# QEDProtocol/plonky2.5

Hardware: NVIDIA B200
Metric: commit Melem/s (2^20x135 LDE+Poseidon Merkle) (higher is better)
Workload: dtype u64 (Goldilocks field, integer + exact fp64 limb arithmetic)

## Files before the change

### plonky2.5_b200/csrc/merkle.cuh

```cuda
#pragma once
#include "poseidon.cuh"

namespace merkle {

__host__ __device__ __forceinline__ uint64_t digest_index(uint32_t layer, uint64_t j) {
    return 2 * (((j >> 1) << (layer + 1)) + (1ULL << layer) - 1) + (j & 1);
}

__device__ __forceinline__ void store_digest(uint64_t* dst, const uint64_t (&s)[poseidon::WIDTH]) {
    ulonglong2* d = reinterpret_cast<ulonglong2*>(dst);
    d[0] = make_ulonglong2(gl::canon(s[0]), gl::canon(s[1]));
    d[1] = make_ulonglong2(gl::canon(s[2]), gl::canon(s[3]));
}

#ifndef LEAF_MIN_BLOCKS
#define LEAF_MIN_BLOCKS 6
#endif
template <int BLOCK>
__global__ void __launch_bounds__(BLOCK, LEAF_MIN_BLOCKS)
leaf_hash_kernel(const uint64_t* __restrict__ leaves, uint32_t pitch, uint32_t leaf_len, uint64_t n_leaves,
                 uint32_t log_sub, uint64_t* __restrict__ digests, uint64_t* __restrict__ cap) {
    uint64_t leaf = (uint64_t)blockIdx.x * BLOCK + threadIdx.x;
    if (leaf >= n_leaves) return;
    const uint64_t* row = leaves + leaf * pitch;
    uint64_t s[poseidon::WIDTH];
#pragma unroll
    for (int i = 0; i < poseidon::WIDTH; i++) s[i] = 0;
    if (leaf_len <= 4) {
#pragma unroll
        for (int i = 0; i < 4; i++)
            if ((uint32_t)i < leaf_len) s[i] = row[i];
    } else {
        const uint32_t n_chunks = (leaf_len + 7) >> 3;
#pragma unroll 1
        for (uint32_t k = 0; k < n_chunks; k++) {
            const ulonglong2* src = reinterpret_cast<const ulonglong2*>(row + 8 * k);
            ulonglong2 v0 = __ldg(src), v1 = __ldg(src + 1), v2 = __ldg(src + 2), v3 = __ldg(src + 3);
            uint64_t in[8] = {v0.x, v0.y, v1.x, v1.y, v2.x, v2.y, v3.x, v3.y};
            const uint32_t rem = leaf_len - 8 * k;
#pragma unroll
            for (int i = 0; i < 8; i++)
                if ((uint32_t)i < rem) s[i] = in[i];
            poseidon::permute(s);
        }
    }
    uint64_t* dst;
    if (log_sub == 0) dst = cap + 4 * leaf;
    else {
        uint64_t L = 1ULL << log_sub, t = leaf >> log_sub, j = leaf & (L - 1);
        dst = digests + 4 * (t * 2 * (L - 1) + digest_index(0, j));
    }
    store_digest(dst, s);
}

template <int BLOCK>
__global__ void __launch_bounds__(BLOCK, LEAF_MIN_BLOCKS)
leaf_absorb_kernel(const uint64_t* __restrict__ leaves, uint32_t pitch, uint32_t leaf_len, uint32_t col0, uint32_t col1, uint64_t n_leaves,
                   uint32_t log_sub, uint64_t* __restrict__ state, uint64_t* __restrict__ digests, uint64_t* __restrict__ cap, int first, int last) {
    const uint64_t leaf = (uint64_t)blockIdx.x * BLOCK + threadIdx.x;
    if (leaf >= n_leaves) return;
    const uint64_t* row = leaves + leaf * pitch;
    uint64_t s[poseidon::WIDTH];
    const bool in_full = leaf_len - col0 >= 8;
#pragma unroll
    for (int i = 0; i < poseidon::WIDTH; i++) s[i] = (first || (i < 8 && in_full)) ? 0 : state[(uint64_t)i * n_leaves + leaf];
#pragma unroll 1
    for (uint32_t k = col0; k < col1; k += 8) {
        const ulonglong2* src = reinterpret_cast<const ulonglong2*>(row + k);
        ulonglong2 v0 = __ldg(src), v1 = __ldg(src + 1), v2 = __ldg(src + 2), v3 = __ldg(src + 3);
        uint64_t in[8] = {v0.x, v0.y, v1.x, v1.y, v2.x, v2.y, v3.x, v3.y};
        const uint32_t rem = leaf_len - k;
#pragma unroll
        for (int i = 0; i < 8; i++)
            if ((uint32_t)i < rem) s[i] = in[i];
        poseidon::permute(s);
    }
    if (!last) {
        const bool out_full = leaf_len - col1 >= 8;
#pragma unroll
        for (int i = 0; i < poseidon::WIDTH; i++)
            if (i >= 8 || !out_full) state[(uint64_t)i * n_leaves + leaf] = s[i];
        return;
    }
    uint64_t* dst;
    if (log_sub == 0) dst = cap + 4 * leaf;
    else {
        uint64_t L = 1ULL << log_sub, t = leaf >> log_sub, j = leaf & (L - 1);
        dst = digests + 4 * (t * 2 * (L - 1) + digest_index(0, j));
    }
    store_digest(dst, s);
}

template <int BLOCK>
__global__ void __launch_bounds__(BLOCK, LEAF_MIN_BLOCKS)
tree_level_kernel(uint64_t* __restrict__ digests, uint64_t* __restrict__ cap, uint32_t layer, uint32_t log_sub,
                  uint64_t n_nodes) {
    uint64_t node = (uint64_t)blockIdx.x * BLOCK + threadIdx.x;
    if (node >= n_nodes) return;
    const uint32_t lw = log_sub - layer;
    const uint64_t t = node >> lw, j = node & ((1ULL << lw) - 1);
    const uint64_t L = 1ULL << log_sub;
    uint64_t* base = digests + 4 * (t * 2 * (L - 1));
    const ulonglong2* ch = reinterpret_cast<const ulonglong2*>(base + 4 * digest_index(layer - 1, 2 * j));
    ulonglong2 a = ch[0], b = ch[1], c = ch[2], d = ch[3];
    uint64_t s[poseidon::WIDTH] = {a.x, a.y, b.x, b.y, c.x, c.y, d.x, d.y, 0, 0, 0, 0};
    poseidon::permute(s);
    uint64_t* dst = (layer == log_sub) ? cap + 4 * t : base + 4 * digest_index(layer, j);
    store_digest(dst, s);
}

__global__ void open_batch_kernel(const uint64_t* __restrict__ leaves, uint32_t pitch, uint32_t leaf_len, const uint64_t* __restrict__ digests,
                                  uint32_t log_sub, const uint64_t* __restrict__ indices, uint32_t n_queries,
                                  uint64_t* __restrict__ out_rows, uint64_t* __restrict__ out_siblings) {
    const uint32_t per_q = leaf_len + 4 * log_sub;
    const uint64_t i = (uint64_t)blockIdx.x * blockDim.x + threadIdx.x;
    if (i >= (uint64_t)n_queries * per_q) return;
    const uint32_t q = (uint32_t)(i / per_q), w = (uint32_t)(i % per_q);
    const uint64_t leaf = indices[q];
    if (w < leaf_len) {
        if (out_rows) out_rows[(size_t)q * leaf_len + w] = leaves[leaf * pitch + w];
        return;
    }
    if (!out_siblings) return;
    const uint32_t layer = (w - leaf_len) >> 2, k = (w - leaf_len) & 3;
    const uint64_t L = 1ULL << log_sub, sub = leaf >> log_sub, j = (leaf & (L - 1)) >> layer;
    out_siblings[((size_t)q * log_sub + layer) * 4 + k] = digests[4 * (sub * 2 * (L - 1) + digest_index(layer, j ^ 1)) + k];
}

__global__ void permute_kernel(uint64_t* __restrict__ states, uint64_t n) {
    uint64_t i = (uint64_t)blockIdx.x * blockDim.x + threadIdx.x;
    if (i >= n) return;
    uint64_t s[poseidon::WIDTH];
#pragma unroll
    for (int k = 0; k < poseidon::WIDTH; k++) s[k] = states[12 * i + k];
    poseidon::permute(s);
#pragma unroll
    for (int k = 0; k < poseidon::WIDTH; k++) states[12 * i + k] = gl::canon(s[k]);
}

__global__ void sponge_absorb_kernel(uint64_t* __restrict__ state12, const uint64_t* __restrict__ groups, uint32_t n_groups) {
    if (blockIdx.x != 0 || threadIdx.x != 0) return;
    uint64_t s[poseidon::WIDTH];
#pragma unroll
    for (int k = 0; k < poseidon::WIDTH; k++) s[k] = state12[k];
#pragma unroll 1
    for (uint32_t g = 0; g < n_groups; g++) {
#pragma unroll
        for (int k = 0; k < poseidon::RATE; k++) s[k] = groups[8 * g + k];
        poseidon::permute(s);
    }
#pragma unroll
    for (int k = 0; k < poseidon::WIDTH; k++) state12[k] = gl::canon(s[k]);
}

__global__ void pow_grind_kernel(const uint64_t* __restrict__ state12, uint32_t pos, uint32_t min_lz, uint64_t base, uint64_t n,
                                 unsigned long long* __restrict__ best) {
    uint64_t i = (uint64_t)blockIdx.x * blockDim.x + threadIdx.x;
    if (i >= n) return;
    const uint64_t w = base + i;
    if (w >= gl::P) return;
    uint64_t s[poseidon::WIDTH];
#pragma unroll
    for (int k = 0; k < poseidon::WIDTH; k++) s[k] = (uint32_t)k == pos ? w : state12[k];
    poseidon::permute(s);
    const uint64_t r = gl::canon(s[poseidon::RATE - 1]);
    const uint32_t lz = r ? (uint32_t)__clzll((long long)r) : 64u;
    if (lz >= min_lz) atomicMin(best, (unsigned long long)w);
}

}
```

### plonky2.5_b200/csrc/poseidon.cuh

```cuda
#pragma once
#include "gl_field.cuh"
#include "poseidon_constants.cuh"

namespace poseidon {

constexpr int WIDTH = 12;
constexpr int RATE = 8;
constexpr int N_FULL_HALF = 4;
constexpr int N_PARTIAL = 22;
constexpr int N_ROUNDS = 30;

#ifndef POSEIDON_SBOX_FORM
#define POSEIDON_SBOX_FORM 0x8
#endif
template <int NEW>
__device__ __forceinline__ uint64_t sbox_sqr(uint64_t x) {
    if (NEW) {
        uint32_t z0, z1, z2, z3;
        gl::mul_words_c(x, x, z0, z1, z2, z3);
        return gl::reduce_words(z0, z1, z2, z3);
    }
    return gl::sqr(x);
}
template <int NEW>
__device__ __forceinline__ void sbox_mul_words(uint64_t a, uint64_t b, uint32_t& z0, uint32_t& z1, uint32_t& z2, uint32_t& z3) {
    if (NEW) gl::mul_words_c(a, b, z0, z1, z2, z3);
    else gl::mul_words(a, b, z0, z1, z2, z3);
}

constexpr double TWO52 = 4503599627370496.0;

__device__ __forceinline__ double biased(uint32_t w) { return __hiloint2double(0x43300000, (int)w); }
__device__ __forceinline__ double limb_to_double(uint32_t w) { return __dsub_rn(biased(w), TWO52); }

__device__ __forceinline__ void sbox7_limbs(uint64_t x, double& lo, double& hi) {
    const uint64_t x2 = sbox_sqr<(POSEIDON_SBOX_FORM >> 0) & 1>(x);
    const uint64_t x4 = sbox_sqr<(POSEIDON_SBOX_FORM >> 1) & 1>(x2);
    uint32_t z0, z1, z2, z3;
    sbox_mul_words<(POSEIDON_SBOX_FORM >> 2) & 1>(x, x2, z0, z1, z2, z3);
    const uint64_t x3 = gl::reduce_words(z0, z1, z2, z3);
    sbox_mul_words<(POSEIDON_SBOX_FORM >> 3) & 1>(x3, x4, z0, z1, z2, z3);
#ifdef POSEIDON_HANDOFF_FP64
    const double d2 = biased(z2);
    lo = __dsub_rn(__dsub_rn(biased(z0), d2), __dsub_rn(biased(z3), TWO52));
    hi = __dsub_rn(__dadd_rn(biased(z1), __dsub_rn(d2, TWO52)), TWO52);
#else
    uint32_t ll, lh, hl, hh;
    asm("{\n\t"
        "sub.cc.u32  %0, %4, %6;\n\t"
        "subc.u32    %1, 0x43300002, 0;\n\t"
        "sub.cc.u32  %0, %0, %7;\n\t"
        "subc.u32    %1, %1, 0;\n\t"
        "add.cc.u32  %2, %5, %6;\n\t"
        "addc.u32    %3, 0x43300000, 0;\n\t"
        "}" : "=&r"(ll), "=&r"(lh), "=&r"(hl), "=&r"(hh) : "r"(z0), "r"(z1), "r"(z2), "r"(z3));
    lo = __dsub_rn(__hiloint2double((int)lh, (int)ll), TWO52 + 8589934592.0);
    hi = __dsub_rn(__hiloint2double((int)hh, (int)hl), TWO52);
#endif
}

__device__ __forceinline__ void mds_limb(const double (&s)[WIDTH], const double* __restrict__ k, double (&o)[WIDTH]) {
    double sp[6], sm[6];
#pragma unroll
    for (int i = 0; i < 6; i++) {
        sp[i] = __dadd_rn(s[i], s[i + 6]);
        sm[i] = __dsub_rn(s[i], s[i + 6]);
    }
    double a[3], b[3];
#pragma unroll
    for (int i = 0; i < 3; i++) {
        a[i] = __dadd_rn(sp[i], sp[i + 3]);
        b[i] = __dsub_rn(sp[i], sp[i + 3]);
    }
    const double S = __dadd_rn(__dadd_rn(a[0], a[1]), a[2]);
    double U[6], V[6];
    {
        double UU[3], UV[3];
#pragma unroll
        for (int j = 0; j < 3; j++) UU[j] = __fma_rn(a[(j + 2) % 3], 16.0, __fma_rn(S, 16.0, k[j]));
        UV[0] = __fma_rn(b[2], 8.0, __fma_rn(b[1], -2.0, __dsub_rn(k[3], b[0])));
        UV[1] = __fma_rn(b[2], -2.0, __fma_rn(b[0], -8.0, __dsub_rn(k[4], b[1])));
        UV[2] = __fma_rn(b[1], -8.0, __fma_rn(b[0], 2.0, __dsub_rn(k[5], b[2])));
#pragma unroll
        for (int j = 0; j < 3; j++) {
            U[j] = __dadd_rn(UU[j], UV[j]);
            U[j + 3] = __dsub_rn(UU[j], UV[j]);
        }
    }
    constexpr double f[6] = {2.0, -4.0, 16.0, 1.0, -1.0, -1.0};
#pragma unroll
    for (int n = 0; n < 6; n++) {
        double acc = k[6 + n];
#pragma unroll
        for (int j = 0; j < 6; j++) acc = __fma_rn(sm[j], (j <= n) ? f[n - j] : -f[6 + n - j], acc);
        V[n] = acc;
    }
    U[0] = __fma_rn(s[0], 4.0, U[0]);
    V[0] = __fma_rn(s[0], 4.0, V[0]);
#pragma unroll
    for (int n = 0; n < 6; n++) {
        o[n] = __dadd_rn(U[n], V[n]);
        o[n + 6] = __dsub_rn(U[n], V[n]);
    }
}

__device__ __forceinline__ uint64_t recombine(double AL, double AH) {
    uint32_t lo, hi;
    asm("{\n\t.reg .u32 u, b1, T, g;\n\t"
        "sub.u32     b1, %5, 0x43300000;\n\t"
        "add.u32     u, %3, b1;\n\t"
        "sub.u32     u, u, 0x43300000;\n\t"
        "add.cc.u32  g, u, %4;\n\t"
        "addc.u32    T, b1, 0;\n\t"
        "addc.u32    g, g, 0;\n\t"
        "sub.cc.u32  %0, %2, T;\n\t"
        "subc.u32    %1, g, 0;\n\t"
        "}" : "=&r"(lo), "=&r"(hi)
            : "r"((uint32_t)__double2loint(AL)), "r"((uint32_t)__double2hiint(AL)), "r"((uint32_t)__double2loint(AH)),
              "r"((uint32_t)__double2hiint(AH)));
    return ((uint64_t)hi << 32) | lo;
}

__device__ __forceinline__ void full_round(uint64_t (&s)[WIDTH], int r) {
    const double* __restrict__ k = POSEIDON_MDS_K[r];
    double lo[WIDTH], hi[WIDTH], AL[WIDTH], AH[WIDTH];
#pragma unroll
    for (int i = 0; i < WIDTH; i++) sbox7_limbs(s[i], lo[i], hi[i]);
    mds_limb(lo, k, AL);
    mds_limb(hi, k + WIDTH, AH);
#pragma unroll
    for (int i = 0; i < WIDTH; i++) s[i] = recombine(AL[i], AH[i]);
}


#if defined(POSEIDON_PARTIAL_V4)
struct Freq {
    double a[3], b[3], m[6];
};

__device__ __forceinline__ void freq_forward(const double (&s)[WIDTH], Freq& f) {
    double sp[6];
    sp[0] = s[6];
    f.m[0] = -s[6];
#pragma unroll
    for (int i = 1; i < 6; i++) {
        sp[i] = __dadd_rn(s[i], s[i + 6]);
        f.m[i] = __dsub_rn(s[i], s[i + 6]);
    }
#pragma unroll
    for (int i = 0; i < 3; i++) {
        f.a[i] = __dadd_rn(sp[i], sp[i + 3]);
        f.b[i] = __dsub_rn(sp[i], sp[i + 3]);
    }
}

__device__ __forceinline__ void freq_round(Freq& f, const double y, const double e) {
    const double d = __dsub_rn(y, e);
    const double a0 = __dadd_rn(f.a[0], d), b0 = __dadd_rn(f.b[0], d), m0 = __dadd_rn(f.m[0], d);
    const double t1 = __dmul_rn(__dadd_rn(f.a[1], f.a[2]), 64.0);
    const double na0 = __fma_rn(y, 8.0, __fma_rn(a0, 64.0, __fma_rn(f.a[2], 64.0, t1)));
    const double na1 = __fma_rn(a0, 128.0, t1);
    const double na2 = __fma_rn(a0, 64.0, __fma_rn(f.a[1], 64.0, t1));
    const double nb0 = __fma_rn(y, 8.0, __fma_rn(b0, -4.0, __fma_rn(f.b[2], 32.0, __dmul_rn(f.b[1], -8.0))));
    const double nb1 = __fma_rn(b0, -32.0, __fma_rn(f.b[1], -4.0, __dmul_rn(f.b[2], -8.0)));
    const double nb2 = __fma_rn(b0, 8.0, __fma_rn(f.b[1], -32.0, __dmul_rn(f.b[2], -4.0)));
    constexpr double g[6] = {4.0, -8.0, 32.0, 2.0, -2.0, -2.0};
    double nm[6];
#pragma unroll
    for (int n = 0; n < 6; n++) {
        double acc = __dmul_rn(f.m[1], (1 <= n) ? g[n - 1] : -g[5 + n]);
#pragma unroll
        for (int j = 2; j < 6; j++) acc = __fma_rn(f.m[j], (j <= n) ? g[n - j] : -g[6 + n - j], acc);
        nm[n] = __fma_rn(m0, g[n], acc);
    }
    nm[0] = __fma_rn(y, 8.0, nm[0]);
    f.a[0] = na0; f.a[1] = na1; f.a[2] = na2;
    f.b[0] = nb0; f.b[1] = nb1; f.b[2] = nb2;
#pragma unroll
    for (int n = 0; n < 6; n++) f.m[n] = nm[n];
}

__device__ __forceinline__ double freq_lane0(const Freq& f) {
    return __fma_rn(__dadd_rn(f.a[0], f.b[0]), 0.25, __dmul_rn(f.m[0], 0.5));
}

__device__ __forceinline__ void normalize_limbs4(double& L, double& H) {
    constexpr double MAGIC4 = 27021597764222976.0;
    constexpr double INV32 = 2.3283064365386963e-10;
    constexpr double B32 = 4294967296.0;
    const double cL = __dsub_rn(__fma_rn(L, INV32, MAGIC4), MAGIC4);
    L = __fma_rn(cL, -B32, L);
    H = __dadd_rn(H, cL);
    const double cH = __dsub_rn(__fma_rn(H, INV32, MAGIC4), MAGIC4);
    H = __fma_rn(cH, -(B32 - 1.0), H);
    L = __dsub_rn(L, cH);
}

__device__ __forceinline__ void partial_rounds(uint64_t (&s)[WIDTH]) {
    Freq FL, FH;
    {
        double l[WIDTH], h[WIDTH];
        l[0] = h[0] = 0.0;
#pragma unroll
        for (int i = 1; i < WIDTH; i++) {
            l[i] = limb_to_double((uint32_t)s[i]);
            h[i] = limb_to_double((uint32_t)(s[i] >> 32));
        }
        freq_forward(l, FL);
        freq_forward(h, FH);
    }
    uint64_t x0 = s[0];
    double eL = 0.0, eH = 0.0;
#pragma unroll 1
    for (int r = 0; r < N_PARTIAL; r++) {
        double yL, yH;
        sbox7_limbs(x0, yL, yH);
        freq_round(FL, yL, eL);
        freq_round(FH, yH, eH);
        if (r & 1) {
#pragma unroll
            for (int i = 0; i < 3; i++) {
                normalize_limbs4(FL.a[i], FH.a[i]);
                normalize_limbs4(FL.b[i], FH.b[i]);
            }
#pragma unroll
            for (int i = 0; i < 6; i++) normalize_limbs4(FL.m[i], FH.m[i]);
        }
        eL = freq_lane0(FL);
        eH = freq_lane0(FH);
        x0 = recombine(__dadd_rn(eL, POSEIDON_PARTIAL4_Q[r][0]), __dadd_rn(eH, POSEIDON_PARTIAL4_Q[r][1]));
    }
    s[0] = x0;
    double l[WIDTH], h[WIDTH];
#pragma unroll
    for (int i = 0; i < 3; i++) {
        const double tpl = __dadd_rn(FL.a[i], FL.b[i]), tml = __dsub_rn(FL.a[i], FL.b[i]);
        const double tph = __dadd_rn(FH.a[i], FH.b[i]), tmh = __dsub_rn(FH.a[i], FH.b[i]);
        const double ml = __dmul_rn(FL.m[i], 0.5), ml3 = __dmul_rn(FL.m[i + 3], 0.5);
        const double mh = __dmul_rn(FH.m[i], 0.5), mh3 = __dmul_rn(FH.m[i + 3], 0.5);
        l[i] = __fma_rn(tpl, 0.25, ml);      l[i + 6] = __fma_rn(tpl, 0.25, -ml);
        l[i + 3] = __fma_rn(tml, 0.25, ml3); l[i + 9] = __fma_rn(tml, 0.25, -ml3);
        h[i] = __fma_rn(tph, 0.25, mh);      h[i + 6] = __fma_rn(tph, 0.25, -mh);
        h[i + 3] = __fma_rn(tmh, 0.25, mh3); h[i + 9] = __fma_rn(tmh, 0.25, -mh3);
    }
#pragma unroll
    for (int i = 1; i < WIDTH; i++)
        s[i] = recombine(__dadd_rn(l[i], POSEIDON_PARTIAL4_TAIL[i - 1][0]), __dadd_rn(h[i], POSEIDON_PARTIAL4_TAIL[i - 1][1]));
}
#else
struct Freq5 {
    double a[3], b[3], p[2], q[4];
};

__device__ __forceinline__ void freq5_forward(const double (&s)[WIDTH], Freq5& f) {
    double sp[6], m[6];
    sp[0] = s[6];
    m[0] = -s[6];
#pragma unroll
    for (int i = 1; i < 6; i++) {
        sp[i] = __dadd_rn(s[i], s[i + 6]);
        m[i] = __dsub_rn(s[i], s[i + 6]);
    }
#pragma unroll
    for (int i = 0; i < 3; i++) {
        f.a[i] = __dadd_rn(sp[i], sp[i + 3]);
        f.b[i] = __dsub_rn(sp[i], sp[i + 3]);
    }
    f.p[0] = __dadd_rn(__dsub_rn(m[0], m[2]), m[4]);
    f.p[1] = __dadd_rn(__dsub_rn(m[1], m[3]), m[5]);
    f.q[0] = __dsub_rn(m[0], m[4]);
    f.q[1] = __dsub_rn(m[1], m[5]);
    f.q[2] = __dadd_rn(m[2], m[4]);
    f.q[3] = __dadd_rn(m[3], m[5]);
}

__device__ __forceinline__ void freq5_round(Freq5& f, const double y, const double e) {
    const double d = __dsub_rn(y, e);
    const double a0 = __dadd_rn(f.a[0], d), b0 = __dadd_rn(f.b[0], d), p0 = __dadd_rn(f.p[0], d), q0 = __dadd_rn(f.q[0], d);
    const double t1 = __dmul_rn(__dadd_rn(f.a[1], f.a[2]), 64.0);
    const double na0 = __fma_rn(y, 8.0, __fma_rn(a0, 64.0, __fma_rn(f.a[2], 64.0, t1)));
    const double na1 = __fma_rn(a0, 128.0, t1);
    const double na2 = __fma_rn(a0, 64.0, __fma_rn(f.a[1], 64.0, t1));
    const double nb0 = __fma_rn(y, 8.0, __fma_rn(b0, -4.0, __fma_rn(f.b[2], 32.0, __dmul_rn(f.b[1], -8.0))));
    const double nb1 = __fma_rn(b0, -32.0, __fma_rn(f.b[1], -4.0, __dmul_rn(f.b[2], -8.0)));
    const double nb2 = __fma_rn(b0, 8.0, __fma_rn(f.b[1], -32.0, __dmul_rn(f.b[2], -4.0)));
    const double np0 = __fma_rn(y, 8.0, __fma_rn(p0, -30.0, __dmul_rn(f.p[1], 12.0)));
    const double np1 = __fma_rn(p0, -12.0, __dmul_rn(f.p[1], -30.0));
    const double nq0 = __fma_rn(y, 8.0, __fma_rn(q0, 6.0, __fma_rn(f.q[2], -30.0, __dmul_rn(f.q[3], 6.0))));
    const double nq1 = __fma_rn(q0, -6.0, __fma_rn(f.q[1], 6.0, __dmul_rn(f.q[3], -30.0)));
    const double nq2 = __fma_rn(q0, 30.0, __fma_rn(f.q[1], -6.0, __fma_rn(f.q[2], 36.0, __dmul_rn(f.q[3], -6.0))));
    const double nq3 = __fma_rn(f.q[1], 30.0, __fma_rn(f.q[2], -6.0, __dmul_rn(f.q[3], 36.0)));
    f.a[0] = na0; f.a[1] = na1; f.a[2] = na2;
    f.b[0] = nb0; f.b[1] = nb1; f.b[2] = nb2;
    f.p[0] = np0; f.p[1] = np1;
    f.q[0] = nq0; f.q[1] = nq1; f.q[2] = nq2; f.q[3] = nq3;
}

constexpr double MAGIC_HALF = 3377699720527872.0;
constexpr double INV6 = 1.0 / 6.0;

__device__ __forceinline__ double third_half(double t) { return __dsub_rn(__fma_rn(t, INV6, MAGIC_HALF), MAGIC_HALF); }

__device__ __forceinline__ double freq5_lane0(const Freq5& f) {
    const double t = __fma_rn(f.q[0], 2.0, __dadd_rn(f.p[0], f.q[2]));
    return __fma_rn(__dadd_rn(f.a[0], f.b[0]), 0.25, third_half(t));
}

__device__ __forceinline__ void normalize_limbs4(double& L, double& H) {
    constexpr double MAGIC4 = 27021597764222976.0;
    constexpr double INV32 = 2.3283064365386963e-10;
    constexpr double B32 = 4294967296.0;
    const double cL = __dsub_rn(__fma_rn(L, INV32, MAGIC4), MAGIC4);
    L = __fma_rn(cL, -B32, L);
    H = __dadd_rn(H, cL);
    const double cH = __dsub_rn(__fma_rn(H, INV32, MAGIC4), MAGIC4);
    H = __fma_rn(cH, -(B32 - 1.0), H);
    L = __dsub_rn(L, cH);
}
__device__ __forceinline__ void normalize_limbs12(double& L, double& H) {
    constexpr double MAGIC = 6755399441055744.0;
    constexpr double C12 = 1.0 / (12.0 * 4294967296.0);
    constexpr double B32 = 4294967296.0;
    const double kL = __dsub_rn(__fma_rn(L, C12, MAGIC), MAGIC);
    L = __fma_rn(kL, -12.0 * B32, L);
    H = __fma_rn(kL, 12.0, H);
    const double kH = __dsub_rn(__fma_rn(H, C12, MAGIC), MAGIC);
    H = __fma_rn(kH, -12.0 * (B32 - 1.0), H);
    L = __fma_rn(kH, -12.0, L);
}

__device__ __forceinline__ void partial_rounds(uint64_t (&s)[WIDTH]) {
    Freq5 FL, FH;
    {
        double l[WIDTH], h[WIDTH];
        l[0] = h[0] = 0.0;
#pragma unroll
        for (int i = 1; i < WIDTH; i++) {
            l[i] = limb_to_double((uint32_t)s[i]);
            h[i] = limb_to_double((uint32_t)(s[i] >> 32));
        }
        freq5_forward(l, FL);
        freq5_forward(h, FH);
    }
    uint64_t x0 = s[0];
    double eL = 0.0, eH = 0.0;
#pragma unroll 1
    for (int r = 0; r < N_PARTIAL; r++) {
        double yL, yH;
        sbox7_limbs(x0, yL, yH);
        freq5_round(FL, yL, eL);
        freq5_round(FH, yH, eH);
        if (r & 1) {
#pragma unroll
            for (int i = 0; i < 3; i++) {
                normalize_limbs4(FL.a[i], FH.a[i]);
                normalize_limbs4(FL.b[i], FH.b[i]);
            }
            normalize_limbs12(FL.p[0], FH.p[0]);
            normalize_limbs12(FL.p[1], FH.p[1]);
#pragma unroll
            for (int i = 0; i < 4; i++) normalize_limbs12(FL.q[i], FH.q[i]);
        }
        eL = freq5_lane0(FL);
        eH = freq5_lane0(FH);
        x0 = recombine(__dadd_rn(eL, POSEIDON_PARTIAL4_Q[r][0]), __dadd_rn(eH, POSEIDON_PARTIAL4_Q[r][1]));
    }
    s[0] = x0;
    double l[WIDTH], h[WIDTH];
    {
        const Freq5* F[2] = {&FL, &FH};
        double* out[2] = {l, h};
#pragma unroll
        for (int k = 0; k < 2; k++) {
            const Freq5& f = *F[k];
            double mh[6];
            mh[0] = third_half(__fma_rn(f.q[0], 2.0, __dadd_rn(f.p[0], f.q[2])));
            mh[1] = third_half(__fma_rn(f.q[1], 2.0, __dadd_rn(f.p[1], f.q[3])));
            mh[2] = third_half(__fma_rn(f.q[2], 2.0, __dsub_rn(f.q[0], f.p[0])));
            mh[3] = third_half(__fma_rn(f.q[3], 2.0, __dsub_rn(f.q[1], f.p[1])));
            mh[4] = third_half(__dadd_rn(__dsub_rn(f.p[0], f.q[0]), f.q[2]));
            mh[5] = third_half(__dadd_rn(__dsub_rn(f.p[1], f.q[1]), f.q[3]));
#pragma unroll
            for (int i = 0; i < 3; i++) {
                const double tp = __dadd_rn(f.a[i], f.b[i]), tm = __dsub_rn(f.a[i], f.b[i]);
                out[k][i] = __fma_rn(tp, 0.25, mh[i]);
                out[k][i + 6] = __fma_rn(tp, 0.25, -mh[i]);
                out[k][i + 3] = __fma_rn(tm, 0.25, mh[i + 3]);
                out[k][i + 9] = __fma_rn(tm, 0.25, -mh[i + 3]);
            }
        }
    }
#pragma unroll
    for (int i = 1; i < WIDTH; i++)
        s[i] = recombine(__dadd_rn(l[i], POSEIDON_PARTIAL4_TAIL[i - 1][0]), __dadd_rn(h[i], POSEIDON_PARTIAL4_TAIL[i - 1][1]));
}
#endif

__device__ __forceinline__ void permute(uint64_t (&s)[WIDTH]) {
#pragma unroll
    for (int i = 0; i < WIDTH; i++) s[i] = gl::add_any_c(s[i], POSEIDON_RC[i]);
#pragma unroll 1
    for (int half = 0; half < 2; half++) {
        const int r0 = half ? N_FULL_HALF + N_PARTIAL : 0;
#pragma unroll 1
        for (int r = r0; r < r0 + N_FULL_HALF; r++) full_round(s, r);
        if (half == 0) partial_rounds(s);
    }
}

}
```

### plonky2.5_b200/csrc/poseidon_constants.cuh

```cuda
#pragma once
#include <stdint.h>
__constant__ uint64_t POSEIDON_RC[360] = {
    0xb585f766f2144405ULL, 0x7746a55f43921ad7ULL, 0xb2fb0d31cee799b4ULL, 0x0f6760a4803427d7ULL,
    0xe10d666650f4e012ULL, 0x8cae14cb07d09bf1ULL, 0xd438539c95f63e9fULL, 0xef781c7ce35b4c3dULL,
    0xcdc4a239b0c44426ULL, 0x277fa208bf337bffULL, 0xe17653a29da578a1ULL, 0xc54302f225db2c76ULL,
    0x86287821f722c881ULL, 0x59cd1a8a41c18e55ULL, 0xc3b919ad495dc574ULL, 0xa484c4c5ef6a0781ULL,
    0x308bbd23dc5416ccULL, 0x6e4a40c18f30c09cULL, 0x9a2eedb70d8f8cfaULL, 0xe360c6e0ae486f38ULL,
    0xd5c7718fbfc647fbULL, 0xc35eae071903ff0bULL, 0x849c2656969c4be7ULL, 0xc0572c8c08cbbbadULL,
    0xe9fa634a21de0082ULL, 0xf56f6d48959a600dULL, 0xf7d713e806391165ULL, 0x8297132b32825dafULL,
    0xad6805e0e30b2c8aULL, 0xac51d9f5fcf8535eULL, 0x502ad7dc18c2ad87ULL, 0x57a1550c110b3041ULL,
    0x66bbd30e6ce0e583ULL, 0x0da2abef589d644eULL, 0xf061274fdb150d61ULL, 0x28b8ec3ae9c29633ULL,
    0x92a756e67e2b9413ULL, 0x70e741ebfee96586ULL, 0x019d5ee2af82ec1cULL, 0x6f6f2ed772466352ULL,
    0x7cf416cfe7e14ca1ULL, 0x61df517b86a46439ULL, 0x85dc499b11d77b75ULL, 0x4b959b48b9c10733ULL,
    0xe8be3e5da8043e57ULL, 0xf5c0bc1de6da8699ULL, 0x40b12cbf09ef74bfULL, 0xa637093ecb2ad631ULL,
    0x3cc3f892184df408ULL, 0x2e479dc157bf31bbULL, 0x6f49de07a6234346ULL, 0x213ce7bede378d7bULL,
    0x5b0431345d4dea83ULL, 0xa2de45780344d6a1ULL, 0x7103aaf94a7bf308ULL, 0x5326fc0d97279301ULL,
    0xa9ceb74fec024747ULL, 0x27f8ec88bb21b1a3ULL, 0xfceb4fda1ded0893ULL, 0xfac6ff1346a41675ULL,
    0x7131aa45268d7d8cULL, 0x9351036095630f9fULL, 0xad535b24afc26bfbULL, 0x4627f5c6993e44beULL,
    0x645cf794b8f1cc58ULL, 0x241c70ed0af61617ULL, 0xacb8e076647905f1ULL, 0x3737e9db4c4f474dULL,
    0xe7ea5e33e75fffb6ULL, 0x90dee49fc9bfc23aULL, 0xd1b1edf76bc09c92ULL, 0x0b65481ba645c602ULL,
    0x99ad1aab0814283bULL, 0x438a7c91d416ca4dULL, 0xb60de3bcc5ea751cULL, 0xc99cab6aef6f58bcULL,
    0x69a5ed92a72ee4ffULL, 0x5e7b329c1ed4ad71ULL, 0x5fc0ac0800144885ULL, 0x32db829239774ecaULL,
    0x0ade699c5830f310ULL, 0x7cc5583b10415f21ULL, 0x85df9ed2e166d64fULL, 0x6604df4fee32bcb1ULL,
    0xeb84f608da56ef48ULL, 0xda608834c40e603dULL, 0x8f97fe408061f183ULL, 0xa93f485c96f37b89ULL,
    0x6704e8ee8f18d563ULL, 0xcee3e9ac1e072119ULL, 0x510d0e65e2b470c1ULL, 0xf6323f486b9038f0ULL,
    0x0b508cdeffa5ceefULL, 0xf2417089e4fb3cbdULL, 0x60e75c2890d15730ULL, 0xa6217d8bf660f29cULL,
    0x7159cd30c3ac118eULL, 0x839b4e8fafead540ULL, 0x0d3f3e5e82920adcULL, 0x8f7d83bddee7bba8ULL,
    0x780f2243ea071d06ULL, 0xeb915845f3de1634ULL, 0xd19e120d26b6f386ULL, 0x016ee53a7e5fecc6ULL,
    0xcb5fd54e7933e477ULL, 0xacb8417879fd449fULL, 0x9c22190be7f74732ULL, 0x5d693c1ba3ba3621ULL,
    0xdcef0797c2b69ec7ULL, 0x3d639263da827b13ULL, 0xe273fd971bc8d0e7ULL, 0x418f02702d227ed5ULL,
    0x8c25fda3b503038cULL, 0x2cbaed4daec8c07cULL, 0x5f58e6afcdd6ddc2ULL, 0x284650ac5e1b0ebaULL,
    0x635b337ee819dab5ULL, 0x9f9a036ed4f2d49fULL, 0xb93e260cae5c170eULL, 0xb0a7eae879ddb76dULL,
    0xd0762cbc8ca6570cULL, 0x34c6efb812b04bf5ULL, 0x40bf0ab5fa14c112ULL, 0xb6b570fc7c5740d3ULL,
    0x5a27b9002de33454ULL, 0xb1a5b165b6d2b2d2ULL, 0x8722e0ace9d1be22ULL, 0x788ee3b37e5680fbULL,
    0x14a726661551e284ULL, 0x98b7672f9ef3b419ULL, 0xbb93ae776bb30e3aULL, 0x28fd3b046380f850ULL,
    0x30a4680593258387ULL, 0x337dc00c61bd9ce1ULL, 0xd5eca244c7a4ff1dULL, 0x7762638264d279bdULL,
    0xc1e434bedeefd767ULL, 0x0299351a53b8ec22ULL, 0xb2d456e4ad251b80ULL, 0x3e9ed1fda49cea0bULL,
    0x2972a92ba450bed8ULL, 0x20216dd77be493deULL, 0xadffe8cf28449ec6ULL, 0x1c4dbb1c4c27d243ULL,
    0x15a16a8a8322d458ULL, 0x388a128b7fd9a609ULL, 0x2300e5d6baedf0fbULL, 0x2f63aa8647e15104ULL,
    0xf1c36ce86ecec269ULL, 0x27181125183970c9ULL, 0xe584029370dca96dULL, 0x4d9bbc3e02f1cfb2ULL,
    0xea35bc29692af6f8ULL, 0x18e21b4beabb4137ULL, 0x1e3b9fc625b554f4ULL, 0x25d64362697828fdULL,
    0x5a3f1bb1c53a9645ULL, 0xdb7f023869fb8d38ULL, 0xb462065911d4e1fcULL, 0x49c24ae4437d8030ULL,
    0xd793862c112b0566ULL, 0xaadd1106730d8febULL, 0xc43b6e0e97b0d568ULL, 0xe29024c18ee6fca2ULL,
    0x5e50c27535b88c66ULL, 0x10383f20a4ff9a87ULL, 0x38e8ee9d71a45af8ULL, 0xdd5118375bf1a9b9ULL,
    0x775005982d74d7f7ULL, 0x86ab99b4dde6c8b0ULL, 0xb1204f603f51c080ULL, 0xef61ac8470250ecfULL,
    0x1bbcd90f132c603fULL, 0x0cd1dabd964db557ULL, 0x11a3ae5beb9d1ec9ULL, 0xf755bfeea585d11dULL,
    0xa3b83250268ea4d7ULL, 0x516306f4927c93afULL, 0xddb4ac49c9efa1daULL, 0x64bb6dec369d4418ULL,
    0xf9cc95c22b4c1fccULL, 0x08d37f755f4ae9f6ULL, 0xeec49b613478675bULL, 0xf143933aed25e0b0ULL,
    0xe4c5dd8255dfc622ULL, 0xe7ad7756f193198eULL, 0x92c2318b87fff9cbULL, 0x739c25f8fd73596dULL,
    0x5636cac9f16dfed0ULL, 0xdd8f909a938e0172ULL, 0xc6401fe115063f5bULL, 0x8ad97b33f1ac1455ULL,
    0x0c49366bb25e8513ULL, 0x0784d3d2f1698309ULL, 0x530fb67ea1809a81ULL, 0x410492299bb01f49ULL,
    0x139542347424b9acULL, 0x9cb0bd5ea1a1115eULL, 0x02e3f615c38f49a1ULL, 0x985d4f4a9c5291efULL,
    0x775b9feafdcd26e7ULL, 0x304265a6384f0f2dULL, 0x593664c39773012cULL, 0x4f0a2e5fb028f2ceULL,
    0xdd611f1000c17442ULL, 0xd8185f9adfea4fd0ULL, 0xef87139ca9a3ab1eULL, 0x3ba71336c34ee133ULL,
    0x7d3a455d56b70238ULL, 0x660d32e130182684ULL, 0x297a863f48cd1f43ULL, 0x90e0a736a751ebb7ULL,
    0x549f80ce550c4fd3ULL, 0x0f73b2922f38bd64ULL, 0x16bf1f73fb7a9c3fULL, 0x6d1f5a59005bec17ULL,
    0x02ff876fa5ef97c4ULL, 0xc5cb72a2a51159b0ULL, 0x8470f39d2d5c900eULL, 0x25abb3f1d39fcb76ULL,
    0x23eb8cc9b372442fULL, 0xd687ba55c64f6364ULL, 0xda8d9e90fd8ff158ULL, 0xe3cbdc7d2fe45ea7ULL,
    0xb9a8c9b3aee52297ULL, 0xc0d28a5c10960bd3ULL, 0x45d7ac9b68f71a34ULL, 0xeeb76e397069e804ULL,
    0x3d06c8bd1514e2d9ULL, 0x9c9c98207cb10767ULL, 0x65700b51aedfb5efULL, 0x911f451539869408ULL,
    0x7ae6849fbc3a0ec6ULL, 0x3bb340eba06afe7eULL, 0xb46e9d8b682ea65eULL, 0x8dcf22f9a3b34356ULL,
    0x77bdaeda586257a7ULL, 0xf19e400a5104d20dULL, 0xc368a348e46d950fULL, 0x9ef1cd60e679f284ULL,
    0xe89cd854d5d01d33ULL, 0x5cd377dc8bb882a2ULL, 0xa7b0fb7883eee860ULL, 0x7684403ec392950dULL,
    0x5fa3f06f4fed3b52ULL, 0x8df57ac11bc04831ULL, 0x2db01efa1e1e1897ULL, 0x54846de4aadb9ca2ULL,
    0xba6745385893c784ULL, 0x541d496344d2c75bULL, 0xe909678474e687feULL, 0xdfe89923f6c9c2ffULL,
    0xece5a71e0cfedc75ULL, 0x5ff98fd5d51fe610ULL, 0x83e8941918964615ULL, 0x5922040b47f150c1ULL,
    0xf97d750e3dd94521ULL, 0x5080d4c2b86f56d7ULL, 0xa7de115b56c78d70ULL, 0x6a9242ac87538194ULL,
    0xf7856ef7f9173e44ULL, 0x2265fc92feb0dc09ULL, 0x17dfc8e4f7ba8a57ULL, 0x9001a64209f21db8ULL,
    0x90004c1371b893c5ULL, 0xb932b7cf752e5545ULL, 0xa0b1df81b6fe59fcULL, 0x8ef1dd26770af2c2ULL,
    0x0541a4f9cfbeed35ULL, 0x9e61106178bfc530ULL, 0xb3767e80935d8af2ULL, 0x0098d5782065af06ULL,
    0x31d191cd5c1466c7ULL, 0x410fefafa319ac9dULL, 0xbdf8f242e316c4abULL, 0x9e8cd55b57637ed0ULL,
    0xde122bebe9a39368ULL, 0x4d001fd58f002526ULL, 0xca6637000eb4a9f8ULL, 0x2f2339d624f91f78ULL,
    0x6d1a7918c80df518ULL, 0xdf9a4939342308e9ULL, 0xebc2151ee6c8398cULL, 0x03cc2ba8a1116515ULL,
    0xd341d037e840cf83ULL, 0x387cb5d25af4afccULL, 0xbba2515f22909e87ULL, 0x7248fe7705f38e47ULL,
    0x4d61e56a525d225aULL, 0x262e963c8da05d3dULL, 0x59e89b094d220ec2ULL, 0x055d5b52b78b9c5eULL,
    0x82b27eb33514ef99ULL, 0xd30094ca96b7ce7bULL, 0xcf5cb381cd0a1535ULL, 0xfeed4db6919e5a7cULL,
    0x41703f53753be59fULL, 0x5eeea940fcde8b6fULL, 0x4cd1f1b175100206ULL, 0x4a20358574454ec0ULL,
    0x1478d361dbbf9facULL, 0x6f02dc07d141875cULL, 0x296a202ed8e556a2ULL, 0x2afd67999bf32ee5ULL,
    0x7acfd96efa95491dULL, 0x6798ba0c0abb2c6dULL, 0x34c6f57b26c92122ULL, 0x5736e1bad206b5deULL,
    0x20057d2a0056521bULL, 0x3dea5bd5d0578bd7ULL, 0x16e50d897d4634acULL, 0x29bff3ecb9b7a6e3ULL,
    0x475cd3205a3bdcdeULL, 0x18a42105c31b7e88ULL, 0x023e7414af663068ULL, 0x15147108121967d7ULL,
    0xe4a3dff1d7d6fef9ULL, 0x01a8d1a588085737ULL, 0x11b4c74eda62beefULL, 0xe587cc0d69a73346ULL,
    0x1ff7327017aa2a6eULL, 0x594e29c42473d06bULL, 0xf6f31db1899b12d5ULL, 0xc02ac5e47312d3caULL,
    0xe70201e960cb78b8ULL, 0x6f90ff3b6a65f108ULL, 0x42747a7245e7fa84ULL, 0xd1f507e43ab749b2ULL,
    0x1c86d265f15750cdULL, 0x3996ce73dd832c1cULL, 0x8e7fba02983224bdULL, 0xba0dec7103255dd4ULL,
    0x9e9cbd781628fc5bULL, 0xdae8645996edd6a5ULL, 0xdebe0853b1a1d378ULL, 0xa49229d24d014343ULL,
    0x7be5b9ffda905e1cULL, 0xa3c95eaec244aa30ULL, 0x0230bca8f4df0544ULL, 0x4135c2bebfe148c6ULL,
    0x166fc0cc438a3c72ULL, 0x3762b59a8ae83efaULL, 0xe8928a4c89114750ULL, 0x2a440b51a4945ee5ULL,
    0x80cefd2b7d99ff83ULL, 0xbb9879c6e61fd62aULL, 0x6e7c8f1a84265034ULL, 0x164bb2de1bbeddc8ULL,
    0xf3c12fe54d5c653bULL, 0x40b9e922ed9771e2ULL, 0x551f5b0fbe7b1840ULL, 0x25032aa7c4cb1811ULL,
    0xaaed34074b164346ULL, 0x8ffd96bbf9c9c81dULL, 0x70fc91eb5937085cULL, 0x7f795e2a5f915440ULL,
    0x4543d9df5476d3cbULL, 0xf172d73e004fc90dULL, 0xdfd1c4febcc81238ULL, 0xbc8dfb627fe558fcULL
};
__constant__ double POSEIDON_MDS_K[30][24] = {
    {5066559299655428.0, 5066559659743249.0, 5066556699189871.0, -1089399876.0, -1622776137.0, 1548346441.0, 4106853828.0, 5532061584.0, -3140763972.0, 1798505532.0, 4879803762.0, 1127383670.0, 5066561963079205.0, 5066555965665590.0, 5066556862397984.0, 773651651.0, 2718007164.0, -1699231876.0, 1979499828.0, 5288372690.0, -2298948592.0, 4036168542.0, -2852664474.0, -7130740196.0},
    {5066556852804611.0, 5066556446044817.0, 5066558547638304.0, -337626365.0, -1172220519.0, -3706207402.0, -6366058114.0, 1111988198.0, -861137422.0, 1827830960.0, 4361752468.0, 4456111766.0, 5066557945527949.0, 5066564524211165.0, 5066559460698950.0, 712695555.0, 735176009.0, 1650591794.0, 3437741496.0, 1323764766.0, 5512208492.0, -1166396514.0, -2709295288.0, 3251402460.0},
    {5066555927494239.0, 5066558885907336.0, 5066557807368505.0, -2991027865.0, 2981522134.0, -1049756671.0, 3056208974.0, -3714830550.0, 4357838562.0, -3125416356.0, -2433160206.0, -7017281788.0, 5066561918919386.0, 5066558682728493.0, 5066559187353083.0, -1395331740.0, -1078598039.0, -5493403485.0, -4187650394.0, 2460537682.0, -4086329278.0, -3274229410.0, 4800476424.0, -573299680.0},
    {5066559228397964.0, 5066557542264310.0, 5066555872615915.0, -2376324612.0, -1662323606.0, 3524208477.0, 1726546048.0, -4826869924.0, -2733605376.0, -4000649748.0, 4826624248.0, 1582325782.0, 5066552763964914.0, 5066558008428212.0, 5066562158163573.0, -1725664302.0, 1247790640.0, -3777178573.0, -438294836.0, -4604276516.0, 1656591196.0, -56492644.0, -1358139220.0, -737434830.0},
    {5066557021692575.0, 5066556050190327.0, 5066557400650228.0, 2315394849.0, 1866464129.0, 4185498598.0, -4814390324.0, 7055467560.0, 3828430370.0, -2554379966.0, -1499949086.0, -3450329078.0, 5066559197829445.0, 5066558172951727.0, 5066557921942677.0, -776410091.0, 1696498155.0, 1500446739.0, -6941809430.0, -3522392894.0, -2638971272.0, -626751340.0, -5212109616.0, -1940155286.0},
    {5066556056291881.0, 5066556653106459.0, 5066552983073941.0, 35515961.0, -516024461.0, -1002111103.0, 2214588378.0, 5592038850.0, 920436998.0, 6167133388.0, -488372392.0, 407959648.0, 5066559511851667.0, 5066558597948127.0, 5066557656340431.0, 750973123.0, 2713197743.0, -6457454883.0, -3809069230.0, 2287435006.0, 1436007696.0, -5797860968.0, -236771488.0, -63231578.0},
    {5066558409836054.0, 5066554209481073.0, 5066560940930315.0, -800642576.0, 65870631.0, 451406639.0, -4365140158.0, 2889814952.0, 3227390282.0, -2802049178.0, 2133049114.0, -6109849792.0, 5066562297966417.0, 5066556662596387.0, 5066557163535506.0, -3619400989.0, 3257507993.0, -1988572934.0, -5146676268.0, 6209086580.0, 1109637296.0, -612439062.0, 2198783586.0, 6784366096.0},
    {5066561674281304.0, 5066558172055953.0, 5066556641480427.0, 610238772.0, 387127155.0, 1493919935.0, -830828796.0, 6858044476.0, 2226066226.0, -3448423548.0, 17296106.0, 2819747848.0, 5066557630146841.0, 5066557739424707.0, 5066556163910145.0, 3249571457.0, -2747908577.0, -2618744877.0, -807543406.0, -3202992982.0, -3742387064.0, -2392678108.0, -302611300.0, -5249954282.0},
    {5066557712151553.0, 5066562046339355.0, 5066559431395555.0, 1671301701.0, -1253073971.0, 3067022573.0, 2054152322.0, 1043576364.0, -3861415144.0, -1407724260.0, 2203285054.0, 443909254.0, 5066559367691526.0, 5066556740436396.0, 5066559391826511.0, -691553766.0, 135360472.0, 1511724599.0, -1093988236.0, -1970364196.0, -3228801778.0, 3506077568.0, -4673246260.0, -7549124300.0},
    {5066557708485256.0, 5066555128366049.0, 5066560493360047.0, -691320816.0, 2111578777.0, 2101657117.0, -5076530060.0, -3050510978.0, 4066471752.0, 6152111708.0, -2665999604.0, 7141383490.0, 5066558871009634.0, 5066557914894006.0, 5066555150714718.0, -2113204912.0, 1709611772.0, -558837460.0, -3679869430.0, 3726378498.0, 4664848934.0, -4043373338.0, -5112199866.0, 5441338158.0},
    {5066556161813290.0, 5066555006500680.0, 5066559294250776.0, -3894090662.0, -1077312464.0, 1929723876.0, -218090492.0, 1586518380.0, -3998605276.0, 4101436144.0, 1532337232.0, -6378976016.0, 5066557612565518.0, 5066559118388195.0, 5066557223702246.0, -3976381594.0, 9313567.0, 941496014.0, 1055393936.0, 4201608966.0, 7889288332.0, 2879421140.0, -1980619272.0, 1931853056.0},
    {5066558332797953.0, 5066553973662536.0, 5066558866235504.0, -2410104093.0, -3295553640.0, -2540055670.0, 4448261492.0, 1047784236.0, 685866242.0, -1366095898.0, -1534282052.0, -2829016090.0, 5066555232013497.0, 5066559873955547.0, 5066558548557214.0, 2897734099.0, 1569304711.0, -4562218144.0, -8186317828.0, 1970744102.0, 476419286.0, -1958688866.0, 8216897168.0, 10544866.0},
    {5066559535718810.0, 5066557615929999.0, 5066556117953027.0, 1562088510.0, 495241823.0, 2653130031.0, 382001264.0, -6752155574.0, -4596028726.0, -7260409132.0, 1338201400.0, 2341335832.0, 5066555454473454.0, 5066556889294574.0, 5066558820072576.0, 2971664366.0, 728018060.0, -2640238620.0, 5553379024.0, -4354249026.0, -3572981260.0, -1664809500.0, 5625957318.0, -4718199704.0},
    {5066561508271697.0, 5066560723232507.0, 5066554088937394.0, -3127110383.0, -1449908755.0, 2789038842.0, 4847295638.0, -5969511480.0, -6234731052.0, -288080496.0, -3680608462.0, 802699424.0, 5066557942798807.0, 5066558671468475.0, 5066553633895061.0, 1376501791.0, 556004627.0, 953339457.0, -3442070626.0, -7387550490.0, -2035020150.0, 1325355720.0, -3774605724.0, 1410020968.0},
    {5066558388961007.0, 5066555786990138.0, 5066553914254597.0, 1285950941.0, 5309337466.0, 279563793.0, -777645312.0, 2968242244.0, -3732589498.0, 5046529950.0, 543998820.0, -818532.0, 5066556406266566.0, 5066560483453105.0, 5066558940157483.0, -1351685922.0, 878340609.0, -4485997335.0, -1283116516.0, -3043251010.0, 3427199052.0, -4129685168.0, 2403524304.0, -1368785390.0},
    {5066561702149965.0, 5066559887700981.0, 5066558108332391.0, -394549233.0, 1619596937.0, 3546345295.0, -144204360.0, 5008750734.0, 3520707022.0, -1313830898.0, -6738617280.0, -2269376696.0, 5066560856721679.0, 5066555002417794.0, 5066560008196230.0, -2558948051.0, 4509245192.0, -139715926.0, -4216152020.0, 3079914050.0, 3990489928.0, 140580418.0, -584094022.0, 651380608.0},
    {5066558422879368.0, 5066559082821248.0, 5066555147354980.0, 365018428.0, 222472004.0, 3012491798.0, -604362112.0, 2622239244.0, 2857086374.0, -905244184.0, -3529624836.0, 2547916086.0, 5066555293014723.0, 5066553862691558.0, 5066556120811623.0, 2934978529.0, 893380736.0, 2621342155.0, 3656600680.0, -1550066638.0, 3446917478.0, 2518265938.0, -1287810314.0, -2206798780.0},
    {5066561961285658.0, 5066557035759023.0, 5066559324209028.0, -2418905996.0, -1373432195.0, 2841778640.0, 5707387702.0, 5277908356.0, 1060878012.0, 1636098002.0, -5817658114.0, 720551344.0, 5066554697767184.0, 5066553956672031.0, 5066556037020021.0, -3258730002.0, 1341457775.0, 2654381359.0, -1808206738.0, -2399155438.0, 1701057780.0, 845976778.0, 1862922264.0, -202889714.0},
    {5066558203608021.0, 5066563275520934.0, 5066554472120231.0, -1129445175.0, 1609509306.0, -535345371.0, 1450384958.0, -327228920.0, -1421955292.0, -4492041988.0, -4632199972.0, 1559791102.0, 5066560805321430.0, 5066558609733820.0, 5066555720249884.0, 1538127946.0, -83417908.0, 10627832.0, 1145836952.0, -2023310700.0, -153539012.0, -7251918200.0, 1539240108.0, 3462445508.0},
    {5066561376674958.0, 5066559225329831.0, 5066555952279238.0, -1159580072.0, 1550849789.0, -4521580244.0, 5835915854.0, -261197056.0, 363696238.0, 3210733274.0, -2457642582.0, -1837415782.0, 5066558040154168.0, 5066560292867945.0, 5066556895237411.0, -1830102164.0, -634739853.0, -4344345803.0, 1568038060.0, 69698812.0, -156968160.0, 4583553900.0, -1152564106.0, 3607523534.0},
    {5066561033086382.0, 5066559857085896.0, 5066560134037051.0, 2269712198.0, -5205662198.0, 2480079859.0, -618944636.0, 2800103998.0, -4030757910.0, -7975454116.0, -1559274138.0, -683762544.0, 5066561460039233.0, 5066555871609882.0, 5066556408602498.0, -2041647625.0, -4591999706.0, 2797265410.0, 7021513440.0, -88889708.0, 5472621200.0, 459146174.0, 6187570708.0, 1614780224.0},
    {5066554006876040.0, 5066557400837517.0, 5066556976365873.0, 2059165654.0, -2270194533.0, -2940477647.0, -4577196950.0, -3583749344.0, 2910124442.0, -369581294.0, 1985221702.0, -4015119568.0, 5066562547099095.0, 5066560842336541.0, 5066552866526657.0, 484261743.0, 1034173827.0, 627401445.0, 1850009290.0, 3696029996.0, -1217386790.0, -1494157636.0, 2745456986.0, -1434236.0},
    {5066561729095438.0, 5066558282794872.0, 5066557302834220.0, 2485092204.0, 2438774184.0, -1355302766.0, 2171448558.0, 4143407112.0, -6119887558.0, -452839466.0, -2906739896.0, 387431762.0, 5066551935437866.0, 5066557606479226.0, 5066558101443511.0, 1485640792.0, 3389251648.0, -2903429149.0, -114816154.0, -1533412842.0, -2221788314.0, -78429694.0, -2806246434.0, 5211989344.0},
    {5066557985544153.0, 5066557941803608.0, 5066559032181864.0, -1698741263.0, 491155846.0, 2916627914.0, -5324044654.0, -2180972190.0, 1811092626.0, -7023982472.0, -6979160374.0, 288964574.0, 5066559785445212.0, 5066560270243090.0, 5066555722983720.0, 2921112854.0, -1788486428.0, 1603142658.0, -3237832458.0, 4624262210.0, 2352754138.0, 1396136202.0, 2599437954.0, 3295686562.0},
    {5066556488212196.0, 5066560432172738.0, 5066556684738309.0, -443580028.0, -891605028.0, -3134048933.0, 1518026564.0, 6435989694.0, -330857916.0, 3855470984.0, 5346134586.0, -5762858298.0, 5066556770214672.0, 5066556391794987.0, 5066558014362321.0, -2280259236.0, -853461581.0, -1375355943.0, -4565963020.0, -4095345370.0, 2226278786.0, 4136207840.0, 7280616944.0, 4813775632.0},
    {5066560767849733.0, 5066560914796777.0, 5066555764040055.0, -2155587357.0, -220977153.0, -218280971.0, 1072467704.0, -3544570464.0, -3022126340.0, -153957450.0, 656274962.0, -4119150154.0, 5066555785809227.0, 5066561231305385.0, 5066555905691521.0, 984334313.0, -5223662627.0, -1743223873.0, 2597586408.0, -6013703554.0, -4544290604.0, -572316766.0, -153591520.0, -3745577502.0},
    {5066560094515061.0, 5066561461361865.0, 5066560882825616.0, 165027655.0, -2371581275.0, 207823328.0, -4759705092.0, 5161109914.0, -1746960620.0, -773539450.0, -1613054292.0, 5507183724.0, 5066561535855110.0, 5066555103965590.0, 5066553603820553.0, -2379672596.0, -3026811842.0, 12193769.0, -5699984394.0, -624850588.0, -2920554882.0, -2222566970.0, 4813251848.0, -3044912560.0},
    {5066556063789336.0, 5066560513533296.0, 5066556128757859.0, 2942837150.0, 667557660.0, 854882817.0, 7126092646.0, 249046436.0, -3294461216.0, -320816818.0, -541985248.0, -3362475878.0, 5066556430983218.0, 5066556371005046.0, 5066553677023377.0, -3860168206.0, 1380468358.0, -850111401.0, -911632424.0, -5423060560.0, -3209633856.0, -1026644868.0, 3556350168.0, 4572545374.0},
    {5066557548762031.0, 5066557453747945.0, 5066559834440522.0, -128048355.0, -783115223.0, 2790306492.0, -6541889936.0, -3103584558.0, 3036815930.0, -4794243198.0, -3101222776.0, -3272460398.0, 5066559760953578.0, 5066556337328146.0, 5066555917840832.0, -5040377860.0, -849538158.0, -2894731084.0, 3244445438.0, 3768599932.0, -2014461800.0, -1714935370.0, 3851270020.0, 6068620716.0},
    {5066549580922880.0, 5066549580922880.0, 5066549580922880.0, 0.0, 0.0, 0.0, 0.0, 0.0, 0.0, 0.0, 0.0, 0.0, 5066549580529664.0, 5066549580529664.0, 5066549580529664.0, 0.0, 0.0, 0.0, 0.0, 0.0, 0.0, 0.0, 0.0, 0.0},
};
__constant__ double POSEIDON_PARTIAL4_Q[22][2] = {
    {6755404383354252.0, 6755401339087428.0},
    {6755411756546256.0, 6755403487607940.0},
    {6755412845655832.0, 6755406928333428.0},
    {6755403331954620.0, 6755402332663988.0},
    {6755403451011900.0, 6755406143336756.0},
    {6755411802142552.0, 6755410276893704.0},
    {6755410397498944.0, 6755407303971060.0},
    {6755406263343860.0, 6755415739843264.0},
    {6755406603547996.0, 6755413694144576.0},
    {6755407416640624.0, 6755403525242376.0},
    {6755416226322408.0, 6755403669613820.0},
    {6755403805615500.0, 6755404173244732.0},
    {6755401502813320.0, 6755403986487704.0},
    {6755405387807020.0, 6755405526100692.0},
    {6755409113491332.0, 6755403673095924.0},
    {6755415630171264.0, 6755413566806668.0},
    {6755408385000620.0, 6755409698924168.0},
    {6755399992403640.0, 6755415499238148.0},
    {6755407909114912.0, 6755406756748932.0},
    {6755400351659448.0, 6755411645865572.0},
    {6755412374333148.0, 6755409931384908.0},
    {6755400348192156.0, 6755410933830524.0},
};
__constant__ double POSEIDON_PARTIAL4_TAIL[11][2] = {
    {6755413960859736.0, 6755411196475692.0},
    {6755401652464580.0, 6755406620509068.0},
    {6755411300162468.0, 6755409780012956.0},
    {6755410294272400.0, 6755416046316252.0},
    {6755409354176364.0, 6755399932835924.0},
    {6755412649279248.0, 6755407536644744.0},
    {6755410388899896.0, 6755405596374180.0},
    {6755411903810008.0, 6755412857106296.0},
    {6755400252699384.0, 6755407245806456.0},
    {6755412125794256.0, 6755406060522364.0},
    {6755408386545996.0, 6755409589943468.0},
};
```

Measured before the change: 1258.

## Skip capacity S-boxes in first full round for tree-node hashing

Tree-level hashing starts with a zero capacity, so the first full round skips the round-constant add and S-box on the capacity lanes. It uses a precomputed MDS constant table that folds in the known capacity values. The partial-round loop is restructured into paired templated steps so normalization is resolved at compile time, and the 1/6 and C12 constants are moved into constant memory. This saves some S-box work per internal node, at the cost of an extra constant table and extra code paths that could change register allocation.

```diff
diff --git a/plonky2.5_b200/csrc/merkle.cuh b/plonky2.5_b200/csrc/merkle.cuh
--- a/plonky2.5_b200/csrc/merkle.cuh
+++ b/plonky2.5_b200/csrc/merkle.cuh
@@ -104,7 +104,7 @@
     const ulonglong2* ch = reinterpret_cast<const ulonglong2*>(base + 4 * digest_index(layer - 1, 2 * j));
     ulonglong2 a = ch[0], b = ch[1], c = ch[2], d = ch[3];
     uint64_t s[poseidon::WIDTH] = {a.x, a.y, b.x, b.y, c.x, c.y, d.x, d.y, 0, 0, 0, 0};
-    poseidon::permute(s);
+    poseidon::permute(s, true);
     uint64_t* dst = (layer == log_sub) ? cap + 4 * t : base + 4 * digest_index(layer, j);
     store_digest(dst, s);
 }
diff --git a/plonky2.5_b200/csrc/poseidon.cuh b/plonky2.5_b200/csrc/poseidon.cuh
--- a/plonky2.5_b200/csrc/poseidon.cuh
+++ b/plonky2.5_b200/csrc/poseidon.cuh
@@ -121,11 +121,17 @@
     return ((uint64_t)hi << 32) | lo;
 }
 
-__device__ __forceinline__ void full_round(uint64_t (&s)[WIDTH], int r) {
-    const double* __restrict__ k = POSEIDON_MDS_K[r];
+__device__ __forceinline__ void full_round(uint64_t (&s)[WIDTH], const double* __restrict__ k, bool zero_cap) {
     double lo[WIDTH], hi[WIDTH], AL[WIDTH], AH[WIDTH];
 #pragma unroll
-    for (int i = 0; i < WIDTH; i++) sbox7_limbs(s[i], lo[i], hi[i]);
+    for (int i = 0; i < RATE; i++) sbox7_limbs(s[i], lo[i], hi[i]);
+    if (zero_cap) {
+#pragma unroll
+        for (int i = RATE; i < WIDTH; i++) lo[i] = hi[i] = 0.0;
+    } else {
+#pragma unroll
+        for (int i = RATE; i < WIDTH; i++) sbox7_limbs(s[i], lo[i], hi[i]);
+    }
     mds_limb(lo, k, AL);
     mds_limb(hi, k + WIDTH, AH);
 #pragma unroll
@@ -297,9 +303,9 @@
 }
 
 constexpr double MAGIC_HALF = 3377699720527872.0;
-constexpr double INV6 = 1.0 / 6.0;
-
-__device__ __forceinline__ double third_half(double t) { return __dsub_rn(__fma_rn(t, INV6, MAGIC_HALF), MAGIC_HALF); }
+__constant__ double POSEIDON_INV6_C12[2] = {1.0 / 6.0, 1.0 / (12.0 * 4294967296.0)};
+
+__device__ __forceinline__ double third_half(double t) { return __dsub_rn(__fma_rn(t, POSEIDON_INV6_C12[0], MAGIC_HALF), MAGIC_HALF); }
 
 __device__ __forceinline__ double freq5_lane0(const Freq5& f) {
     const double t = __fma_rn(f.q[0], 2.0, __dadd_rn(f.p[0], f.q[2]));
@@ -319,7 +325,7 @@
 }
 __device__ __forceinline__ void normalize_limbs12(double& L, double& H) {
     constexpr double MAGIC = 6755399441055744.0;
-    constexpr double C12 = 1.0 / (12.0 * 4294967296.0);
+    const double C12 = POSEIDON_INV6_C12[1];
     constexpr double B32 = 4294967296.0;
     const double kL = __dsub_rn(__fma_rn(L, C12, MAGIC), MAGIC);
     L = __fma_rn(kL, -12.0 * B32, L);
@@ -329,6 +335,30 @@
     L = __fma_rn(kH, -12.0, L);
 }
 
+__device__ __forceinline__ void freq5_normalize(Freq5& FL, Freq5& FH) {
+#pragma unroll
+    for (int i = 0; i < 3; i++) {
+        normalize_limbs4(FL.a[i], FH.a[i]);
+        normalize_limbs4(FL.b[i], FH.b[i]);
+    }
+    normalize_limbs12(FL.p[0], FH.p[0]);
+    normalize_limbs12(FL.p[1], FH.p[1]);
+#pragma unroll
+    for (int i = 0; i < 4; i++) normalize_limbs12(FL.q[i], FH.q[i]);
+}
+
+template <bool NORM>
+__device__ __forceinline__ void partial_round(uint64_t& x0, Freq5& FL, Freq5& FH, double& eL, double& eH, const double* __restrict__ q) {
+    double yL, yH;
+    sbox7_limbs(x0, yL, yH);
+    freq5_round(FL, yL, eL);
+    freq5_round(FH, yH, eH);
+    if (NORM) freq5_normalize(FL, FH);
+    eL = freq5_lane0(FL);
+    eH = freq5_lane0(FH);
+    x0 = recombine(__dadd_rn(eL, q[0]), __dadd_rn(eH, q[1]));
+}
+
 __device__ __forceinline__ void partial_rounds(uint64_t (&s)[WIDTH]) {
     Freq5 FL, FH;
     {
@@ -345,25 +375,9 @@
     uint64_t x0 = s[0];
     double eL = 0.0, eH = 0.0;
 #pragma unroll 1
-    for (int r = 0; r < N_PARTIAL; r++) {
-        double yL, yH;
-        sbox7_limbs(x0, yL, yH);
-        freq5_round(FL, yL, eL);
-        freq5_round(FH, yH, eH);
-        if (r & 1) {
-#pragma unroll
-            for (int i = 0; i < 3; i++) {
-                normalize_limbs4(FL.a[i], FH.a[i]);
-                normalize_limbs4(FL.b[i], FH.b[i]);
-            }
-            normalize_limbs12(FL.p[0], FH.p[0]);
-            normalize_limbs12(FL.p[1], FH.p[1]);
-#pragma unroll
-            for (int i = 0; i < 4; i++) normalize_limbs12(FL.q[i], FH.q[i]);
-        }
-        eL = freq5_lane0(FL);
-        eH = freq5_lane0(FH);
-        x0 = recombine(__dadd_rn(eL, POSEIDON_PARTIAL4_Q[r][0]), __dadd_rn(eH, POSEIDON_PARTIAL4_Q[r][1]));
+    for (int r = 0; r < N_PARTIAL; r += 2) {
+        partial_round<false>(x0, FL, FH, eL, eH, POSEIDON_PARTIAL4_Q[r]);
+        partial_round<true>(x0, FL, FH, eL, eH, POSEIDON_PARTIAL4_Q[r + 1]);
     }
     s[0] = x0;
     double l[WIDTH], h[WIDTH];
@@ -396,14 +410,18 @@
 }
 #endif
 
-__device__ __forceinline__ void permute(uint64_t (&s)[WIDTH]) {
-#pragma unroll
-    for (int i = 0; i < WIDTH; i++) s[i] = gl::add_any_c(s[i], POSEIDON_RC[i]);
+__device__ __forceinline__ void permute(uint64_t (&s)[WIDTH], bool zero_cap = false) {
+#pragma unroll
+    for (int i = 0; i < WIDTH; i++)
+        if (i < RATE || !zero_cap) s[i] = gl::add_any_c(s[i], POSEIDON_RC[i]);
 #pragma unroll 1
     for (int half = 0; half < 2; half++) {
         const int r0 = half ? N_FULL_HALF + N_PARTIAL : 0;
 #pragma unroll 1
-        for (int r = r0; r < r0 + N_FULL_HALF; r++) full_round(s, r);
+        for (int r = r0; r < r0 + N_FULL_HALF; r++) {
+            const bool zc = zero_cap && r == 0;
+            full_round(s, zc ? POSEIDON_MDS_K0_ZC : POSEIDON_MDS_K[r], zc);
+        }
         if (half == 0) partial_rounds(s);
     }
 }
diff --git a/plonky2.5_b200/csrc/poseidon_constants.cuh b/plonky2.5_b200/csrc/poseidon_constants.cuh
--- a/plonky2.5_b200/csrc/poseidon_constants.cuh
+++ b/plonky2.5_b200/csrc/poseidon_constants.cuh
@@ -161,3 +161,4 @@
     {6755412125794256.0, 6755406060522364.0},
     {6755408386545996.0, 6755409589943468.0},
 };
+__constant__ double POSEIDON_MDS_K0_ZC[24] = {5066842818157332.0, 5066788995573185.0, 5066817546337135.0, 9322337078.0, 20611412284.0, 30802976289.0, 59647160245.0, 50009337906.0, -12365616268.0, 1460696496.0, -42188165147.0, -26390137567.0, 5066828153132565.0, 5066755519113158.0, 5066751599255968.0, 9527928924.0, 21060710006.0, 8442470475.0, 18499939202.0, 49282528894.0, -10004285907.0, 8262540004.0, -54358679578.0, -43453959039.0};
```

Result: no change. 1265, median of 6 (+0.6%).
